# Netflix/metaflow

Measured on AMD Instinct MI355X. Metric: tokens/sec, higher is better.
Workload: dtype bf16; 1 GPU; model=llama3-8b, global_batch=8, seq_len=4096, parallelism=dp1

## Files before the change

### metaflow_amd/ops/csrc/attention.hip

```cpp

#include "common.h"

#define ATT_D 128

typedef __attribute__((ext_vector_type(16))) float f16f;

DEV f16f mfma32(bf16x8 a, bf16x8 b, f16f c) {
  return __builtin_amdgcn_mfma_f32_32x32x16_bf16(a, b, c, 0, 0, 0);
}

struct WaveCoord {
  int wid, lane, l32, hi;
};

DEV WaveCoord wave_coord() {
  WaveCoord c;
  c.wid = threadIdx.x / WAVE;
  c.lane = threadIdx.x & (WAVE - 1);
  c.l32 = c.lane & 31;
  c.hi = c.lane >> 5;
  return c;
}

DEV int c_row(int r, int hi) { return (r & 3) + 8 * (r >> 2) + 4 * hi; }

DEV unsigned int pack_bf2(float lo, float hi) {
  union { __hip_bfloat162 h; unsigned int u; } c;
  c.h = __float22bfloat162_rn(make_float2(lo, hi));
  return c.u;
}

template <int NT>
DEV void col_to_afrags(const f16f* st, bf16x8* pa, int hi) {
  unsigned int pk[NT * 8], xp[NT * 8];
#pragma unroll
  for (int t = 0; t < NT; ++t)
#pragma unroll
    for (int j2 = 0; j2 < 8; ++j2)
      pk[t * 8 + j2] = pack_bf2(st[t][j2 * 2], st[t][j2 * 2 + 1]);
#pragma unroll
  for (int i = 0; i < NT * 8; ++i) xp[i] = __shfl_xor(pk[i], 32, WAVE);
#pragma unroll
  for (int ks = 0; ks < NT * 2; ++ks) {
    union {
      unsigned int w[4];
      bf16x8 v;
    } u;
    if (hi == 0) {
      u.w[0] = pk[4 * ks];
      u.w[1] = pk[4 * ks + 1];
      u.w[2] = xp[4 * ks];
      u.w[3] = xp[4 * ks + 1];
    } else {
      u.w[0] = xp[4 * ks + 2];
      u.w[1] = xp[4 * ks + 3];
      u.w[2] = pk[4 * ks + 2];
      u.w[3] = pk[4 * ks + 3];
    }
    pa[ks] = u.v;
  }
}


template <int ROWS, int BLOCK>
DEV void stage_panel(short* dst, const short* src,
                     long long src_row_stride) {
  constexpr int TOT = ROWS * 16;
#pragma unroll
  for (int it = 0; it < (TOT + BLOCK - 1) / BLOCK; ++it) {
    const int idx = it * BLOCK + threadIdx.x;
    if (idx < TOT) {
      const int r = idx % ROWS, c8 = idx / ROWS;
      bf16x8 v = *(const bf16x8*)(src + r * src_row_stride + c8 * 8);
      *(bf16x8*)(dst + (c8 >> 1) * (ROWS * 16) + r * 16 + (c8 & 1) * 8) =
          v;
    }
  }
}

template <int ROWS>
DEV bf16x8 frag8_panel(const short* tile, int row, int d0) {
  return *(const bf16x8*)(tile + (d0 >> 4) * (ROWS * 16) + row * 16
                          + (d0 & 15));
}

DEV unsigned long long tr_read(const short* lds_ptr) {
  unsigned int addr = (unsigned int)(unsigned long long)lds_ptr;
  unsigned long long out;
  asm volatile("ds_read_b64_tr_b16 %0, %1" : "=v"(out) : "v"(addr));
  return out;
}

union BFrag {
  unsigned long long u[2];
  bf16x8 v;
};

template <int ROWS>
DEV void tr_load_bfrags(BFrag bfr[4], const short* tile, int row0,
                        int lane, int hi) {
  const int tr_lane_off = (((lane >> 2) & 3) * 16) + (lane & 3) * 4;
  const int tr_panel = ((lane >> 4) & 1) * (ROWS * 16);
#pragma unroll
  for (int n = 0; n < 4; ++n) {
    const int base = n * 2 * (ROWS * 16) + tr_panel
                     + (row0 + hi * 8) * 16 + tr_lane_off;
    bfr[n].u[0] = tr_read(tile + base);
    bfr[n].u[1] = tr_read(tile + base + 4 * 16);
  }
}

DEV void put_elem(short* p, float x) { *p = f2bf(x); }
DEV void put_elem(float* p, float x) { *p = x; }

template <bool ROW_SCALE, typename T>
DEV void store_acc_tile(T* dst, long long off0, int row0, const f16f acc[4],
                        int l32, int hi, float lane_scale = 1.f) {
#pragma unroll
  for (int r = 0; r < 16; ++r) {
    const int row_local = c_row(r, hi);
    float f = 1.f;
    if (ROW_SCALE) f = __shfl(lane_scale, row_local + 32 * hi, WAVE);
    const long long obase = off0 + (long long)(row0 + row_local) * ATT_D;
#pragma unroll
    for (int n = 0; n < 4; ++n)
      put_elem(dst + obase + n * 32 + l32,
               ROW_SCALE ? acc[n][r] * f : acc[n][r]);
  }
}


template <int BLOCK>
__global__ __launch_bounds__(512) void attn_fwd_v2_kernel(
    const short* __restrict__ q, const short* __restrict__ k,
    const short* __restrict__ v, short* __restrict__ o,
    float* __restrict__ lse, int B, int H, int Hkv, int S, float scale,
    int causal) {
  constexpr int BQ = 256, BKV = 64;
  __shared__ short kp[2][BKV * ATT_D];
  __shared__ short vp[2][BKV * ATT_D];

  const int qb = blockIdx.x;
  const int h = blockIdx.y;
  const int b = blockIdx.z;
  const int hk = h / (H / Hkv);
  const WaveCoord c = wave_coord();
  const int wid = c.wid, lane = c.lane, l32 = c.l32, hi = c.hi;

  const int my_qrow = qb * BQ + wid * 32 + l32;
  const long long hoff = ((long long)b * H + h) * S;
  const long long qoff = (hoff + qb * BQ) * ATT_D;
  const long long kvoff0 = ((long long)b * Hkv + hk) * S * ATT_D;

  bf16x8 q_reg[8];
  {
    const short* qrow = q + (hoff + my_qrow) * ATT_D;
#pragma unroll
    for (int s = 0; s < 8; ++s)
      q_reg[s] = *(const bf16x8*)(qrow + s * 16 + hi * 8);
  }

  float m_run = -INFINITY;
  float l_run = 0.f;
  f16f acc_o[4];
#pragma unroll
  for (int n = 0; n < 4; ++n) acc_o[n] = (f16f){};

  const int tid = threadIdx.x;
  bf16x8 stg_k[2], stg_v[2];
  int stg_r[2], stg_c8[2];
#pragma unroll
  for (int u = 0; u < 2; ++u) {
    const int idx = u * BLOCK + tid;
    stg_r[u] = idx / 16;
    stg_c8[u] = idx % 16;
  }

#define MFX_STAGE_LOAD(jj)                                               \
  {                                                                      \
    const short* kb_ = k + kvoff0 + (long long)(jj) * BKV * ATT_D;       \
    const short* vb_ = v + kvoff0 + (long long)(jj) * BKV * ATT_D;       \
    _Pragma("unroll") for (int u = 0; u < 2; ++u) {                      \
      stg_k[u] = *(const bf16x8*)(kb_ + stg_r[u] * ATT_D + stg_c8[u] * 8);\
      stg_v[u] = *(const bf16x8*)(vb_ + stg_r[u] * ATT_D + stg_c8[u] * 8);\
    }                                                                    \
  }

#define MFX_STAGE_WRITE(buf)                                             \
  {                                                                      \
    _Pragma("unroll") for (int u = 0; u < 2; ++u) {                      \
      const int pel_ = (stg_c8[u] >> 1) * (BKV * 16) + stg_r[u] * 16     \
                       + (stg_c8[u] & 1) * 8;                            \
      *(bf16x8*)(kp[buf] + pel_) = stg_k[u];                             \
      *(bf16x8*)(vp[buf] + pel_) = stg_v[u];                             \
    }                                                                    \
  }

  const int kv_tiles =
      causal ? (qb * BQ + BQ) / BKV : S / BKV;
  MFX_STAGE_LOAD(0);
  MFX_STAGE_WRITE(0);
  __syncthreads();
  for (int j = 0; j < kv_tiles; ++j) {
    const int cur = j & 1;
    if (j + 1 < kv_tiles) MFX_STAGE_LOAD(j + 1);

    const bool active = !causal || (j * BKV <= qb * BQ + wid * 32 + 31);
    if (active) {

    f16f st[2];
#pragma unroll
    for (int t = 0; t < 2; ++t) {
      st[t] = (f16f){};
#pragma unroll
      for (int s = 0; s < 8; ++s) {
        bf16x8 kf = frag8_panel<BKV>(kp[cur], t * 32 + l32,
                                     s * 16 + hi * 8);
        st[t] = mfma32(kf, q_reg[s], st[t]);
      }
    }

    const bool diag = causal && (j * BKV + BKV > qb * BQ);
    float pmax = -INFINITY;
#pragma unroll
    for (int t = 0; t < 2; ++t) {
#pragma unroll
      for (int r = 0; r < 16; ++r) {
        float sv = st[t][r] * scale;
        if (diag) {
          const int kvg = j * BKV + t * 32 + c_row(r, hi);
          if (kvg > my_qrow) sv = -INFINITY;
        }
        st[t][r] = sv;
        pmax = fmaxf(pmax, sv);
      }
    }
    pmax = fmaxf(pmax, __shfl_xor(pmax, 32, WAVE));
    const float newm = fmaxf(m_run, pmax);
    const float rescale = __expf(m_run - newm);
    m_run = newm;

    float psum = 0.f;
#pragma unroll
    for (int t = 0; t < 2; ++t)
#pragma unroll
      for (int r = 0; r < 16; ++r) {
        float e = __expf(st[t][r] - newm);
        st[t][r] = e;
        psum += e;
      }
    psum += __shfl_xor(psum, 32, WAVE);
    l_run = l_run * rescale + psum;

    {
#pragma unroll
      for (int r = 0; r < 16; ++r) {
        const float f = __shfl(rescale, c_row(r, hi) + 32 * hi, WAVE);
#pragma unroll
        for (int n = 0; n < 4; ++n) acc_o[n][r] *= f;
      }
    }

    bf16x8 pa[4];
    col_to_afrags<2>(st, pa, hi);

    {
      const int tr_lane_off = (((lane >> 2) & 3) * 16) + (lane & 3) * 4;
      const int tr_panel = ((lane >> 4) & 1) * (BKV * 16);
#pragma unroll
      for (int ks = 0; ks < 4; ++ks) {
        BFrag bfr[4];
#pragma unroll
        for (int n = 0; n < 4; ++n) {
          const int base = n * 2 * (BKV * 16) + tr_panel
                           + (ks * 16 + hi * 8) * 16 + tr_lane_off;
          bfr[n].u[0] = tr_read(vp[cur] + base);
          bfr[n].u[1] = tr_read(vp[cur] + base + 4 * 16);
        }
        asm volatile("s_waitcnt lgkmcnt(0)");
        __builtin_amdgcn_sched_barrier(0);
#pragma unroll
        for (int n = 0; n < 4; ++n)
          acc_o[n] = mfma32(pa[ks], bfr[n].v, acc_o[n]);
      }
    }
    }

    if (j + 1 < kv_tiles) MFX_STAGE_WRITE(cur ^ 1);
    __syncthreads();
  }
#undef MFX_STAGE_LOAD
#undef MFX_STAGE_WRITE

  float inv_l = 1.f / l_run;
  store_acc_tile<true>(o, qoff, wid * 32, acc_o, l32, hi, inv_l);
  if (hi == 0)
    lse[hoff + my_qrow] = m_run + __logf(l_run);
}

__global__ void attn_bwd_delta_kernel(const short* __restrict__ dout,
                                      const short* __restrict__ o,
                                      float* __restrict__ delta,
                                      long long rows) {
  const int lane = threadIdx.x & (WAVE - 1);
  const int wid = threadIdx.x / WAVE;
  const long long row = (long long)blockIdx.x * (blockDim.x / WAVE) + wid;
  if (row >= rows) return;
  const short* dr = dout + row * ATT_D;
  const short* orow = o + row * ATT_D;
  float s = bf2f(dr[lane]) * bf2f(orow[lane])
            + bf2f(dr[lane + 64]) * bf2f(orow[lane + 64]);
  s = wave_sum(s);
  if (lane == 0) delta[row] = s;
}


template <int BLOCK>
__global__ __launch_bounds__(512) void attn_bwd_dq_v2_kernel(
    const short* __restrict__ q, const short* __restrict__ k,
    const short* __restrict__ v, const short* __restrict__ dout,
    const float* __restrict__ lse, const float* __restrict__ delta,
    short* __restrict__ dq, int B, int H, int Hkv, int S, float scale,
    int causal) {
  constexpr int BQ = 256, BKV = 64;
  __shared__ short kp[BKV * ATT_D];
  __shared__ short vp[BKV * ATT_D];

  const int qb = blockIdx.x;
  const int h = blockIdx.y;
  const int b = blockIdx.z;
  const int hk = h / (H / Hkv);
  const int wid = threadIdx.x / WAVE;
  const int lane = threadIdx.x & (WAVE - 1);
  const int l32 = lane & 31;
  const int hi = lane >> 5;

  const int my_qrow = qb * BQ + wid * 32 + l32;
  const long long hoff = ((long long)b * H + h) * S;
  const long long qoff = (hoff + qb * BQ) * ATT_D;
  const long long kvoff0 = ((long long)b * Hkv + hk) * S * ATT_D;

  bf16x8 q_reg[8], do_reg[8];
  {
    const short* qrow = q + (hoff + my_qrow) * ATT_D;
    const short* drow = dout + (hoff + my_qrow) * ATT_D;
#pragma unroll
    for (int s = 0; s < 8; ++s) {
      q_reg[s] = *(const bf16x8*)(qrow + s * 16 + hi * 8);
      do_reg[s] = *(const bf16x8*)(drow + s * 16 + hi * 8);
    }
  }
  const float my_lse = lse[hoff + my_qrow];
  const float my_del = delta[hoff + my_qrow];

  f16f acc_dq[4];
#pragma unroll
  for (int n = 0; n < 4; ++n) acc_dq[n] = (f16f){};

  const int kv_tiles = causal ? (qb * BQ + BQ) / BKV : S / BKV;
  for (int j = 0; j < kv_tiles; ++j) {
    __syncthreads();
    stage_panel<BKV, BLOCK>(kp, k + kvoff0 + (long long)j * BKV * ATT_D,
                            ATT_D);
    stage_panel<BKV, BLOCK>(vp, v + kvoff0 + (long long)j * BKV * ATT_D,
                            ATT_D);
    __syncthreads();
    if (causal && j * BKV > qb * BQ + wid * 32 + 31) continue;

#pragma unroll
    for (int t = 0; t < 2; ++t) {
      f16f st = (f16f){}, dpt = (f16f){};
#pragma unroll
      for (int s = 0; s < 8; ++s) {
        bf16x8 kf = frag8_panel<BKV>(kp, t * 32 + l32, s * 16 + hi * 8);
        bf16x8 vf = frag8_panel<BKV>(vp, t * 32 + l32, s * 16 + hi * 8);
        st = mfma32(kf, q_reg[s], st);
        dpt = mfma32(vf, do_reg[s], dpt);
      }
#pragma unroll
      for (int r = 0; r < 16; ++r) {
        const int kvg = j * BKV + t * 32 + c_row(r, hi);
        float p = 0.f;
        if (!causal || kvg <= my_qrow)
          p = __expf(st[r] * scale - my_lse);
        st[r] = p * (dpt[r] - my_del) * scale;
      }
      bf16x8 pa[2];
      col_to_afrags<1>(&st, pa, hi);
#pragma unroll
      for (int ks = 0; ks < 2; ++ks) {
        BFrag bfr[4];
        tr_load_bfrags<BKV>(bfr, kp, t * 32 + ks * 16, lane, hi);
        asm volatile("s_waitcnt lgkmcnt(0)");
        __builtin_amdgcn_sched_barrier(0);
#pragma unroll
        for (int n = 0; n < 4; ++n)
          acc_dq[n] = mfma32(pa[ks], bfr[n].v, acc_dq[n]);
      }
    }
  }

#pragma unroll
  for (int r = 0; r < 16; ++r) {
    const int row_local = (r & 3) + 8 * (r >> 2) + 4 * hi;
    const long long obase =
        qoff + (long long)(wid * 32 + row_local) * ATT_D;
#pragma unroll
    for (int n = 0; n < 4; ++n)
      dq[obase + n * 32 + l32] = f2bf(acc_dq[n][r]);
  }
}


DEV void acc_to_bfrags(const f16f& x, bf16x8* pb) {
#pragma unroll
  for (int s = 0; s < 2; ++s) {
    unsigned int w[4];
#pragma unroll
    for (int i = 0; i < 4; ++i)
      w[i] = pack_bf2(x[8 * s + 2 * i], x[8 * s + 2 * i + 1]);
    union {
      unsigned int w[4];
      bf16x8 v;
    } u;
#pragma unroll
    for (int i = 0; i < 2; ++i) {
      auto r = __builtin_amdgcn_permlane32_swap(w[i], w[2 + i], false,
                                                false);
      u.w[i] = r[0];
      u.w[2 + i] = r[1];
    }
    pb[s] = u.v;
  }
}

DEV void lds_wave_fence() {
  __builtin_amdgcn_fence(__ATOMIC_RELEASE, "wavefront");
  __builtin_amdgcn_wave_barrier();
  __builtin_amdgcn_fence(__ATOMIC_ACQUIRE, "wavefront");
}

DEV void store_acc_tile_t(float* dst, long long off0, float* tw,
                          const f16f acc[4], int l32, int hi) {
#pragma unroll
  for (int n = 0; n < 4; ++n) {
#pragma unroll
    for (int r = 0; r < 16; ++r) {
      const int dl = (r & 3) + 8 * (r >> 2) + 4 * hi;
      tw[l32 * 32 + (dl ^ l32)] = acc[n][r];
    }
    lds_wave_fence();
#pragma unroll
    for (int i = 0; i < 16; ++i) {
      const int row = 2 * i + hi;
      dst[off0 + (long long)row * ATT_D + n * 32 + l32] =
          tw[row * 32 + (l32 ^ row)];
    }
    lds_wave_fence();
  }
}

extern __shared__ __attribute__((aligned(16))) short dkdv_v_img[];
#define DKDV_DYN_LDS (256 * ATT_D * 2)

template <int BLOCK>
__global__ __launch_bounds__(512) void attn_bwd_dkdv_v2_kernel(
    const short* __restrict__ q, const short* __restrict__ k,
    const short* __restrict__ v, const short* __restrict__ dout,
    const float* __restrict__ lse, const float* __restrict__ delta,
    float* __restrict__ dk_part, float* __restrict__ dv_part,
    int B, int H, int Hkv, int S, float scale, int causal) {
  constexpr int BKVB = 256, BQ2 = 64;
  __shared__ short qp[BQ2 * ATT_D];
  __shared__ short dop[BQ2 * ATT_D];
  __shared__ float lse_s[BQ2];
  __shared__ float del_s[BQ2];

  const int kvb = blockIdx.x;
  const int h = blockIdx.y;
  const int b = blockIdx.z;
  const int G = H / Hkv;
  const int hk = h / G;
  const int wid = threadIdx.x / WAVE;
  const int lane = threadIdx.x & (WAVE - 1);
  const int l32 = lane & 31;
  const int hi = lane >> 5;

  const int my_kvrow = kvb * BKVB + wid * 32 + l32;
  const long long kvoff =
      (((long long)b * Hkv + hk) * S + kvb * BKVB) * ATT_D;

  bf16x8 kr[8];
  short* vimg = dkdv_v_img + wid * (32 * ATT_D) + lane * 8;
  {
    const short* krow = k + kvoff + (long long)(wid * 32 + l32) * ATT_D;
    const short* vrow = v + kvoff + (long long)(wid * 32 + l32) * ATT_D;
#pragma unroll
    for (int s = 0; s < 8; ++s) {
      kr[s] = *(const bf16x8*)(krow + s * 16 + hi * 8);
      *(bf16x8*)(vimg + s * 512) = *(const bf16x8*)(vrow + s * 16 + hi * 8);
    }
#pragma unroll
    for (int s = 0; s < 8; ++s) asm volatile("" : "+v"(kr[s]));
  }

  f16f acc_dk[4], acc_dv[4];
#pragma unroll
  for (int n = 0; n < 4; ++n) {
    acc_dk[n] = (f16f){};
    acc_dv[n] = (f16f){};
  }

  const long long hoff = ((long long)b * H + h) * S;
  const int jq0 = causal ? (kvb * BKVB) / BQ2 : 0;
  const int nq = S / BQ2;
  for (int jq = jq0; jq < nq; ++jq) {
    __syncthreads();
    const short* qsrc = q + (hoff + (long long)jq * BQ2) * ATT_D;
    const short* dsrc = dout + (hoff + (long long)jq * BQ2) * ATT_D;
    stage_panel<BQ2, BLOCK>(qp, qsrc, ATT_D);
    stage_panel<BQ2, BLOCK>(dop, dsrc, ATT_D);
    if (threadIdx.x < BQ2) {
      lse_s[threadIdx.x] = lse[hoff + jq * BQ2 + threadIdx.x];
      del_s[threadIdx.x] = delta[hoff + jq * BQ2 + threadIdx.x];
    }
    __syncthreads();
    if (causal && jq * BQ2 + BQ2 - 1 < kvb * BKVB + wid * 32) continue;

#pragma unroll
    for (int t = 0; t < 2; ++t) {
      f16f st = (f16f){}, dpt = (f16f){};
#pragma unroll
      for (int s = 0; s < 8; ++s) {
        bf16x8 qf = frag8_panel<BQ2>(qp, t * 32 + l32, s * 16 + hi * 8);
        bf16x8 df = frag8_panel<BQ2>(dop, t * 32 + l32, s * 16 + hi * 8);
        bf16x8 vf = *(const bf16x8*)(vimg + s * 512);
        st = mfma32(qf, kr[s], st);
        dpt = mfma32(df, vf, dpt);
      }
#pragma unroll
      for (int g = 0; g < 4; ++g) {
        const int q0l = t * 32 + g * 8 + 4 * hi;
        const f32x4 lv = *(const f32x4*)&lse_s[q0l];
        const f32x4 dl = *(const f32x4*)&del_s[q0l];
#pragma unroll
        for (int j = 0; j < 4; ++j) {
          const int r = g * 4 + j;
          const int qrg = jq * BQ2 + q0l + j;
          float p = 0.f;
          if (!causal || qrg >= my_kvrow)
            p = __expf(st[r] * scale - lv[j]);
          st[r] = p;
          dpt[r] = p * (dpt[r] - dl[j]) * scale;
        }
      }
      bf16x8 pb[2], pbk[2];
      acc_to_bfrags(st, pb);
      BFrag bfr[2][4];
      const int tr_lane_off = (((lane >> 2) & 3) * 16) + (lane & 3) * 4;
      const int tr_panel = ((lane >> 4) & 1) * (BQ2 * 16);
      const short* g_tile[4] = {dop, dop, qp, qp};
      int g_q0[4];
      g_q0[0] = t * 32;
      g_q0[1] = t * 32 + 16;
      g_q0[2] = t * 32;
      g_q0[3] = t * 32 + 16;
#pragma unroll
      for (int n = 0; n < 4; ++n) {
        const int base = n * 2 * (BQ2 * 16) + tr_panel
                         + (g_q0[0] + hi * 8) * 16 + tr_lane_off;
        bfr[0][n].u[0] = tr_read(g_tile[0] + base);
        bfr[0][n].u[1] = tr_read(g_tile[0] + base + 4 * 16);
      }
      acc_to_bfrags(dpt, pbk);
#pragma unroll
      for (int g = 0; g < 4; ++g) {
        const int cur = g & 1;
        if (g < 3) {
#pragma unroll
          for (int n = 0; n < 4; ++n) {
            const int base = n * 2 * (BQ2 * 16) + tr_panel
                             + (g_q0[g + 1] + hi * 8) * 16 + tr_lane_off;
            bfr[cur ^ 1][n].u[0] = tr_read(g_tile[g + 1] + base);
            bfr[cur ^ 1][n].u[1] = tr_read(g_tile[g + 1] + base + 4 * 16);
          }
          asm volatile("s_waitcnt lgkmcnt(8)");
        } else {
          asm volatile("s_waitcnt lgkmcnt(0)");
        }
        __builtin_amdgcn_sched_barrier(0);
        const bf16x8 bop = (g < 2) ? pb[g] : pbk[g - 2];
        f16f* acc = (g < 2) ? acc_dv : acc_dk;
#pragma unroll
        for (int n = 0; n < 4; ++n)
          acc[n] = mfma32(bfr[cur][n].v, bop, acc[n]);
      }
    }
  }

  __syncthreads();
  float* tw = (float*)(wid < 4 ? qp : dop) + (wid & 3) * 1024;
  const long long poff =
      (hoff + (long long)kvb * BKVB + wid * 32) * ATT_D;
  store_acc_tile_t(dk_part, poff, tw, acc_dk, l32, hi);
  store_acc_tile_t(dv_part, poff, tw, acc_dv, l32, hi);
}

__global__ void dkdv_reduce_kernel(const float* __restrict__ dk_part,
                                   const float* __restrict__ dv_part,
                                   short* __restrict__ dk,
                                   short* __restrict__ dv,
                                   long long n4_kv, int G,
                                   long long head_elems) {
  const long long stride = (long long)gridDim.x * blockDim.x;
  for (long long i4 = (long long)blockIdx.x * blockDim.x + threadIdx.x;
       i4 < n4_kv; i4 += stride) {
    const long long i = i4 * 4;
    const long long slot = i / head_elems;
    const long long rem = i - slot * head_elems;
    const float* kp = dk_part + slot * G * head_elems + rem;
    const float* vp = dv_part + slot * G * head_elems + rem;
    f32x4 ks = *(const f32x4*)kp;
    f32x4 vs = *(const f32x4*)vp;
    for (int g = 1; g < G; ++g) {
      const f32x4 k2 = *(const f32x4*)(kp + (long long)g * head_elems);
      const f32x4 v2 = *(const f32x4*)(vp + (long long)g * head_elems);
#pragma unroll
      for (int j = 0; j < 4; ++j) {
        ks[j] += k2[j];
        vs[j] += v2[j];
      }
    }
    bf16x4 ko, vo;
// ... 10 lines not shown
```

### metaflow_amd/ops/csrc/mfx_hip.hip

```cpp

#include <torch/extension.h>
#include <hip/hip_runtime.h>
#include <c10/hip/HIPStream.h>

#include <vector>

#include "elementwise.hip"
#include "adam.hip"
#include "cross_entropy.hip"
#include "attention.hip"
#include "append.hip"
#include "decode.hip"
#include "paged.hip"
#include "append_paged.hip"
#include "debug_kernels.hip"

namespace {

constexpr int kBlock = 256;
constexpr int kGridCap = 2048;

inline hipStream_t cur_stream() {
  return c10::hip::getCurrentHIPStream().stream();
}
// ... 144 lines not shown
  auto du = torch::empty_like(u);
  long long n8 = g.numel() / 8;
  swiglu_bwd_kernel<<<grid_for(n8), kBlock, 0, cur_stream()>>>(
      bf(g), bf(u), bf(dy), bfm(dg), bfm(du), n8);
  HIP_CHECK_KERNEL();
  return {dg, du};
}

std::vector<torch::Tensor> swiglu_gu_fwd(torch::Tensor gu) {
  check_bf16(gu, "gu");
  const int I2 = gu.size(-1);
  TORCH_CHECK(I2 % 16 == 0, "fused swiglu needs 2I % 16 == 0");
  const int I = I2 / 2;
  const long long rows = gu.numel() / I2;
  auto sizes = gu.sizes().vec();
  sizes.back() = I;
  auto y = torch::empty(sizes, gu.options());
  long long total = rows * (I / 8);
  swiglu_gu_fwd_kernel<<<grid_for(total), kBlock, 0, cur_stream()>>>(
      bf(gu), bfm(y), rows, I);
  HIP_CHECK_KERNEL();
  return {y};
}

torch::Tensor swiglu_gu_bwd(torch::Tensor gu, torch::Tensor dy) {
  const int I = gu.size(-1) / 2;
  const long long rows = gu.numel() / (2 * I);
  auto dgu = torch::empty_like(gu);
  long long total = rows * (I / 8);
  swiglu_gu_bwd_kernel<<<grid_for(total), kBlock, 0, cur_stream()>>>(
      bf(gu), bf(dy.contiguous()), bfm(dgu), rows, I);
  HIP_CHECK_KERNEL();
  return dgu;
}

torch::Tensor decode_tokens_u16(torch::Tensor x) {
  TORCH_CHECK(x.is_cuda() && x.is_contiguous());
  TORCH_CHECK(x.scalar_type() == torch::kUInt8, "pass raw bytes (uint8)");
  TORCH_CHECK(x.numel() % 16 == 0,
              "token buffer must hold a multiple of 8 uint16 tokens");
  const long long n = x.numel() / 2;
  auto y = torch::empty({n}, x.options().dtype(torch::kInt64));
  decode_tokens_u16_kernel<<<grid_for(n / 8), kBlock, 0, cur_stream()>>>(
      reinterpret_cast<const unsigned short*>(x.data_ptr()),
      reinterpret_cast<long long*>(y.data_ptr<int64_t>()), n / 8);
  HIP_CHECK_KERNEL();
  return y;
}

torch::Tensor quant_e4m3(torch::Tensor x, double scale) {
  check_bf16(x, "x");
  TORCH_CHECK(x.numel() % 8 == 0, "quant_e4m3 needs numel % 8 == 0");
  auto y = torch::empty_like(x, x.options().dtype(torch::kUInt8));
  long long n8 = x.numel() / 8;
  quant_e4m3_kernel<<<grid_for(n8), kBlock, 0, cur_stream()>>>(
      bf(x), y.data_ptr<unsigned char>(), (float)scale, n8);
  HIP_CHECK_KERNEL();
  return y;
}

torch::Tensor quant_e5m2(torch::Tensor x, double scale) {
  check_bf16(x, "x");
  TORCH_CHECK(x.numel() % 8 == 0, "quant_e5m2 needs numel % 8 == 0");
  auto y = torch::empty_like(x, x.options().dtype(torch::kUInt8));
  long long n8 = x.numel() / 8;
  quant_e5m2_kernel<<<grid_for(n8), kBlock, 0, cur_stream()>>>(
      bf(x), y.data_ptr<unsigned char>(), (float)scale, n8);
  HIP_CHECK_KERNEL();
  return y;
}

torch::Tensor add_bf16(torch::Tensor a, torch::Tensor b) {
  check_bf16(a, "a");
  TORCH_CHECK(a.numel() % 8 == 0);
  auto y = torch::empty_like(a);
  long long n8 = a.numel() / 8;
  add_bf16_kernel<<<grid_for(n8), kBlock, 0, cur_stream()>>>(
      bf(a), bf(b), bfm(y), n8);
  HIP_CHECK_KERNEL();
  return y;
}

void adamw(torch::Tensor p, torch::Tensor g, torch::Tensor m, torch::Tensor v,
           c10::optional<torch::Tensor> master, double lr, double beta1,
           double beta2, double eps, double weight_decay, long step,
           double grad_scale) {
  const long long n = p.numel();
  float bias_c1 = 1.f / (1.f - powf((float)beta1, (float)step));
  float bias_c2 = 1.f / (1.f - powf((float)beta2, (float)step));
  if (p.scalar_type() == torch::kBFloat16) {
    TORCH_CHECK(n % 4 == 0, "bf16 adamw requires numel % 4 == 0");
    float* master_ptr =
        master.has_value() ? master->data_ptr<float>() : nullptr;
    adamw_kernel<<<grid_for(n / 4), kBlock, 0, cur_stream()>>>(
        bfm(p), bf(g), m.data_ptr<float>(), v.data_ptr<float>(), master_ptr,
        n, (float)lr, (float)beta1, (float)beta2, (float)eps,
        (float)weight_decay, bias_c1, bias_c2, (float)grad_scale);
    HIP_CHECK_KERNEL();
  } else {
    adamw_f32_kernel<<<grid_for(n), kBlock, 0, cur_stream()>>>(
        p.data_ptr<float>(), g.data_ptr<float>(), m.data_ptr<float>(),
        v.data_ptr<float>(), n, (float)lr, (float)beta1, (float)beta2,
        (float)eps, (float)weight_decay, bias_c1, bias_c2,
        (float)grad_scale);
    HIP_CHECK_KERNEL();
  }
}

std::vector<torch::Tensor> cross_entropy_fwd(torch::Tensor logits,
                                             torch::Tensor targets,
                                             long ignore_index) {
  check_bf16(logits, "logits");
  const int V = logits.size(-1);
  const long long N = logits.numel() / V;
  auto loss = torch::empty({N}, logits.options().dtype(torch::kFloat32));
  auto rmax = torch::empty({N}, logits.options().dtype(torch::kFloat32));
  auto rlse = torch::empty({N}, logits.options().dtype(torch::kFloat32));
  int grid = (int)std::min<long long>(N, kGridCap);
  cross_entropy_fwd_kernel<kBlock><<<grid, kBlock, 0, cur_stream()>>>(
      bf(logits), reinterpret_cast<const long long*>(targets.data_ptr<int64_t>()), loss.data_ptr<float>(),
      rmax.data_ptr<float>(), rlse.data_ptr<float>(), N, V,
      (long long)ignore_index);
  HIP_CHECK_KERNEL();
  return {loss, rlse};
}

torch::Tensor cross_entropy_bwd(torch::Tensor logits, torch::Tensor targets,
                                torch::Tensor row_lse, torch::Tensor dloss,
                                long ignore_index) {
  const int V = logits.size(-1);
  const long long N = logits.numel() / V;
  auto dlogits = torch::empty_like(logits);
  int grid = (int)std::min<long long>(N, kGridCap);
  cross_entropy_bwd_kernel<kBlock><<<grid, kBlock, 0, cur_stream()>>>(
      bf(logits), reinterpret_cast<const long long*>(targets.data_ptr<int64_t>()), row_lse.data_ptr<float>(),
      dloss.data_ptr<float>(), bfm(dlogits), N, V, (long long)ignore_index);
  HIP_CHECK_KERNEL();
  return dlogits;
}

std::vector<torch::Tensor> attn_fwd(torch::Tensor q, torch::Tensor k,
                                    torch::Tensor v, double scale,
                                    bool causal) {
  check_bf16(q, "q");
  check_bf16(k, "k");
  check_bf16(v, "v");
  const int B = q.size(0), H = q.size(1), S = q.size(2), D = q.size(3);
  const int Hkv = k.size(1);
  TORCH_CHECK(D == 128, "attention requires head dim 128");
  TORCH_CHECK(S % 256 == 0, "attention kernel requires seqlen % 256 == 0");
  TORCH_CHECK(H % Hkv == 0, "GQA requires H % Hkv == 0");
  auto o = torch::empty_like(q);
  auto lse = torch::empty({B, H, S}, q.options().dtype(torch::kFloat32));
  dim3 grid(S / 256, H, B);
  attn_fwd_v2_kernel<512><<<grid, 512, 0, cur_stream()>>>(
      bf(q), bf(k), bf(v), bfm(o), lse.data_ptr<float>(), B, H, Hkv, S,
      (float)scale, causal ? 1 : 0);
  HIP_CHECK_KERNEL();
  return {o, lse};
}

std::vector<torch::Tensor> attn_bwd(torch::Tensor q, torch::Tensor k,
                                    torch::Tensor v, torch::Tensor o,
                                    torch::Tensor dout, torch::Tensor lse,
                                    double scale, bool causal) {
  check_bf16(q, "q");
  check_bf16(k, "k");
  check_bf16(v, "v");
  check_bf16(o, "o");
  check_bf16(dout, "dout");
  const int B = q.size(0), H = q.size(1), S = q.size(2), D = q.size(3);
  const int Hkv = k.size(1);
  TORCH_CHECK(D == 128, "attention requires head dim 128");
  TORCH_CHECK(S % 256 == 0, "attention kernel requires seqlen % 256 == 0");
  TORCH_CHECK(H % Hkv == 0, "GQA requires H % Hkv == 0");
  TORCH_CHECK(lse.is_cuda() && lse.scalar_type() == torch::kFloat32 &&
                  lse.is_contiguous(),
              "lse must be contiguous fp32 on GPU");
  TORCH_CHECK(lse.dim() == 3 && lse.size(0) == B && lse.size(1) == H &&
                  lse.size(2) == S,
              "lse must have shape [B,H,S]");
  auto dq = torch::empty_like(q);
  auto dk = torch::empty_like(k);
  auto dv = torch::empty_like(v);
  auto f32opts = q.options().dtype(torch::kFloat32);
  auto delta = torch::empty({B, H, S}, f32opts);
  auto dk_part = torch::empty({B, H, S, 128}, f32opts);
  auto dv_part = torch::empty({B, H, S, 128}, f32opts);
  const int icausal = causal ? 1 : 0;
  const dim3 grid(S / 256, H, B);

  {
    const long long rows = (long long)B * H * S;
    const int rows_per_block = kBlock / 64;
    const long long blocks = (rows + rows_per_block - 1) / rows_per_block;
    attn_bwd_delta_kernel<<<(int)blocks, kBlock, 0, cur_stream()>>>(
        bf(dout), bf(o), delta.data_ptr<float>(), rows);
    HIP_CHECK_KERNEL();
  }
  {
    static bool lds_set[64] = {};
    int dev_id = 0;
    TORCH_CHECK(hipGetDevice(&dev_id) == hipSuccess && dev_id < 64,
                "attn_bwd: hipGetDevice failed");
    if (!lds_set[dev_id]) {
      hipError_t e = hipFuncSetAttribute(
          reinterpret_cast<const void*>(&attn_bwd_dkdv_v2_kernel<512>),
          hipFuncAttributeMaxDynamicSharedMemorySize, DKDV_DYN_LDS);
      TORCH_CHECK(e == hipSuccess, "attn_bwd: cannot raise dynamic LDS: ",
                  hipGetErrorString(e));
      lds_set[dev_id] = true;
    }
  }
  attn_bwd_dkdv_v2_kernel<512><<<grid, 512, DKDV_DYN_LDS, cur_stream()>>>(
      bf(q), bf(k), bf(v), bf(dout), lse.data_ptr<float>(),
      delta.data_ptr<float>(), dk_part.data_ptr<float>(),
      dv_part.data_ptr<float>(), B, H, Hkv, S, (float)scale, icausal);
  HIP_CHECK_KERNEL();
  {
    const long long n4_kv = (long long)B * Hkv * S * 128 / 4;
    const long long head_elems = (long long)S * 128;
    int blocks = (int)std::min<long long>(
        (n4_kv + kBlock - 1) / kBlock, kGridCap);
    dkdv_reduce_kernel<<<blocks, kBlock, 0, cur_stream()>>>(
        dk_part.data_ptr<float>(), dv_part.data_ptr<float>(), bfm(dk),
        bfm(dv), n4_kv, H / Hkv, head_elems);
    HIP_CHECK_KERNEL();
  }
  attn_bwd_dq_v2_kernel<512><<<grid, 512, 0, cur_stream()>>>(
      bf(q), bf(k), bf(v), bf(dout), lse.data_ptr<float>(),
      delta.data_ptr<float>(), bfm(dq), B, H, Hkv, S, (float)scale,
      icausal);
  HIP_CHECK_KERNEL();
  return {dq, dk, dv};
}

torch::Tensor attn_decode_varlen(torch::Tensor q, torch::Tensor kc,
                                 torch::Tensor vc, torch::Tensor lengths,
                                 long max_len, double scale) {
  check_bf16(q, "q");
  check_bf16(kc, "kc");
  check_bf16(vc, "vc");
  const int B = q.size(0), H = q.size(1);
  const int Hkv = kc.size(1), Lmax = kc.size(2);
  TORCH_CHECK(q.size(2) == 1 && q.size(3) == 128,
              "decode expects q [B,H,1,128]");
  TORCH_CHECK(kc.size(3) == 128 && max_len >= 1 && max_len <= Lmax);
  TORCH_CHECK(H % Hkv == 0);
  TORCH_CHECK(lengths.is_cuda() &&
              lengths.scalar_type() == torch::kInt32 &&
              lengths.numel() == B, "lengths must be int32 [B] on GPU");
  int splits = (int)std::max<long>(1, 1024 / ((long)B * H));
  splits = (int)std::min<long>(splits, (max_len + 255) / 256);
  splits = std::max(splits, 1);
  auto f32 = q.options().dtype(torch::kFloat32);
  auto o_part = torch::empty({splits, B, H, 128}, f32);
  auto ml_part = torch::empty({splits, B, H, 2}, f32);
  auto o = torch::empty_like(q);
  dim3 grid(splits, H, B);
  attn_decode_partial_kernel<<<grid, 256, 0, cur_stream()>>>(
      bf(q), bf(kc), bf(vc), lengths.data_ptr<int>(),
      o_part.data_ptr<float>(), ml_part.data_ptr<float>(), B, H, Hkv,
      Lmax, splits, (float)scale);
  HIP_CHECK_KERNEL();
  attn_decode_merge_kernel<<<B * H, 64, 0, cur_stream()>>>(
      o_part.data_ptr<float>(), ml_part.data_ptr<float>(), bfm(o), B, H,
      splits);
  HIP_CHECK_KERNEL();
  return o;
}

torch::Tensor attn_decode(torch::Tensor q, torch::Tensor kc,
                          torch::Tensor vc, long L, double scale) {
  auto lengths = torch::full({q.size(0)}, (long)L,
                             q.options().dtype(torch::kInt32));
  return attn_decode_varlen(q, kc, vc, lengths, L, scale);
}

torch::Tensor attn_append(torch::Tensor q, torch::Tensor kc,
                          torch::Tensor vc, torch::Tensor pos,
                          long max_len, double scale) {
  check_bf16(q, "q");
  check_bf16(kc, "kc");
  check_bf16(vc, "vc");
  TORCH_CHECK(q.dim() == 4 && q.size(3) == 128 && q.size(2) >= 1,
              "append expects q [B,H,Sq,128]");
  const int B = q.size(0), H = q.size(1), Sq = q.size(2);
  TORCH_CHECK(kc.dim() == 4 && kc.size(0) == B && kc.size(3) == 128,
              "append expects k_cache [B,Hkv,Lmax,128]");
  TORCH_CHECK(vc.sizes() == kc.sizes(),
              "k_cache and v_cache must have the same shape");
  const int Hkv = kc.size(1), Lmax = kc.size(2);
  TORCH_CHECK(H % Hkv == 0, "GQA requires H % Hkv == 0");
  TORCH_CHECK(max_len >= 1 && max_len <= Lmax,
              "max_len must be in [1, Lmax]");
  TORCH_CHECK(pos.is_cuda() && pos.scalar_type() == torch::kInt32 &&
              pos.numel() == B && pos.is_contiguous(),
              "pos must be int32 [B] on GPU");
  const bool small = Sq <= 32;
  const int bq = small ? 32 : 128;
  const int q_tiles = (Sq + bq - 1) / bq;
  const long wgs = (long)B * H * q_tiles;
  int splits = (int)std::max<long>(1, (small ? 1024 : 512) / wgs);
  splits = (int)std::min<long>(splits, (max_len + 255) / 256);
  splits = std::max(splits, 1);
  auto o = torch::empty_like(q);
  auto f32 = q.options().dtype(torch::kFloat32);
  torch::Tensor o_part, ml_part;
  float* o_part_p = nullptr;
  float* ml_part_p = nullptr;
  if (splits > 1) {
    o_part = torch::empty({splits, B, H, Sq, 128}, f32);
    ml_part = torch::empty({splits, B, H, Sq, 2}, f32);
    o_part_p = o_part.data_ptr<float>();
    ml_part_p = ml_part.data_ptr<float>();
  }
  dim3 grid(q_tiles * splits, H, B);
  if (small)
    attn_append_kernel<1><<<grid, 64, 0, cur_stream()>>>(
        bf(q), bf(kc), bf(vc), pos.data_ptr<int>(), bfm(o), o_part_p,
        ml_part_p, B, H, Hkv, Sq, Lmax, splits, (float)scale);
  else
    attn_append_kernel<4><<<grid, 256, 0, cur_stream()>>>(
        bf(q), bf(kc), bf(vc), pos.data_ptr<int>(), bfm(o), o_part_p,
        ml_part_p, B, H, Hkv, Sq, Lmax, splits, (float)scale);
  HIP_CHECK_KERNEL();
  if (splits > 1) {
    const long long R = (long long)B * H * Sq;
    attn_append_merge_kernel<<<(int)((R + 3) / 4), 256, 0, cur_stream()>>>(
        o_part_p, ml_part_p, bfm(o), R, splits);
    HIP_CHECK_KERNEL();
  }
  return o;
}

void check_page_pool(const torch::Tensor& kp, const torch::Tensor& vp) {
  check_bf16(kp, "k_pages");
  check_bf16(vp, "v_pages");
  TORCH_CHECK(kp.dim() == 4 && kp.size(2) == PG_ROWS && kp.size(3) == PG_D,
              "page pool must be [num_pages, Hkv, 64, 128]");
  TORCH_CHECK(vp.sizes() == kp.sizes(),
              "k_pages and v_pages must have the same shape");
}

void check_block_table(const torch::Tensor& table, int B) {
  TORCH_CHECK(table.is_cuda() && table.scalar_type() == torch::kInt32 &&
              table.dim() == 2 && table.size(0) == B &&
              table.is_contiguous(),
              "block_table must be contiguous int32 [B, pages_per_seq] "
              "on GPU");
}

torch::Tensor attn_decode_paged(torch::Tensor q, torch::Tensor kp,
                                torch::Tensor vp, torch::Tensor table,
                                torch::Tensor lengths, long max_len,
                                double scale) {
  check_bf16(q, "q");
  check_page_pool(kp, vp);
  TORCH_CHECK(q.dim() == 4 && q.size(2) == 1 && q.size(3) == PG_D,
              "paged decode expects q [B,H,1,128]");
  const int B = q.size(0), H = q.size(1);
  const int num_pages = kp.size(0), Hkv = kp.size(1);
  TORCH_CHECK(H % Hkv == 0, "GQA requires H % Hkv == 0");
  check_block_table(table, B);
  const int table_stride = table.size(1);
  TORCH_CHECK(max_len >= 1 && max_len <= (long)table_stride * PG_ROWS,
              "max_len must be in [1, 64 * pages_per_seq]");
  TORCH_CHECK(lengths.is_cuda() &&
              lengths.scalar_type() == torch::kInt32 &&
              lengths.numel() == B && lengths.is_contiguous(),
              "lengths must be int32 [B] on GPU");
  int splits = (int)std::max<long>(1, 1024 / ((long)B * H));
  splits = (int)std::min<long>(splits, (max_len + 255) / 256);
  splits = (int)std::min<long>(splits,
                               (max_len + PG_ROWS - 1) / PG_ROWS);
  splits = std::max(splits, 1);
  auto f32 = q.options().dtype(torch::kFloat32);
  auto o_part = torch::empty({splits, B, H, 128}, f32);
  auto ml_part = torch::empty({splits, B, H, 2}, f32);
  auto o = torch::empty_like(q);
  dim3 grid(splits, H, B);
  attn_decode_paged_partial_kernel<<<grid, 256, 0, cur_stream()>>>(
// ... 179 lines not shown
```

Baseline: 18550 tokens/s.

## Reorder attention grids heavy-first, double-buffer dQ KV staging, transpose MFMA outputs

Flattens the attention grids to 1D and maps blocks so causal query tiles with the most KV work launch first, which is meant to reduce tail imbalance. The dQ backward kernel gains register-prefetched, double-buffered K/V staging through a second dynamic-LDS buffer, so global loads overlap compute and one barrier per tile is dropped. The forward and dQ kernels swap MFMA operands so P lands in B-fragments via permlane32_swap. That removes per-row shuffles for the rescale and half-wave reductions. Outputs are written as bf16 through an LDS transpose for coalesced 16-byte stores. In exchange the dQ kernel uses more LDS and the block-index mapping becomes more complex.

```diff
diff --git a/metaflow_amd/ops/csrc/attention.hip b/metaflow_amd/ops/csrc/attention.hip
--- a/metaflow_amd/ops/csrc/attention.hip
+++ b/metaflow_amd/ops/csrc/attention.hip
@@ -129,6 +129,98 @@
   }
 }
 
+DEV void acc_to_bfrags(const f16f& x, bf16x8* pb) {
+#pragma unroll
+  for (int s = 0; s < 2; ++s) {
+    unsigned int w[4];
+#pragma unroll
+    for (int i = 0; i < 4; ++i)
+      w[i] = pack_bf2(x[8 * s + 2 * i], x[8 * s + 2 * i + 1]);
+    union {
+      unsigned int w[4];
+      bf16x8 v;
+    } u;
+#pragma unroll
+    for (int i = 0; i < 2; ++i) {
+      auto r = __builtin_amdgcn_permlane32_swap(w[i], w[2 + i], false,
+                                                false);
+      u.w[i] = r[0];
+      u.w[2 + i] = r[1];
+    }
+    pb[s] = u.v;
+  }
+}
+
+DEV float half_pair_max(float x) {
+  const unsigned int u = __float_as_uint(x);
+  auto r = __builtin_amdgcn_permlane32_swap(u, u, false, false);
+  return fmaxf(__uint_as_float(r[0]), __uint_as_float(r[1]));
+}
+
+DEV float half_pair_sum(float x) {
+  const unsigned int u = __float_as_uint(x);
+  auto r = __builtin_amdgcn_permlane32_swap(u, u, false, false);
+  return __uint_as_float(r[0]) + __uint_as_float(r[1]);
+}
+
+DEV void lds_wave_fence() {
+  __builtin_amdgcn_fence(__ATOMIC_RELEASE, "wavefront");
+  __builtin_amdgcn_wave_barrier();
+  __builtin_amdgcn_fence(__ATOMIC_ACQUIRE, "wavefront");
+}
+
+template <int NB, bool ROW_SCALE>
+DEV void store_acc_tile_t_bf16(short* dst, long long off0, short* tw,
+                               const f16f acc[4], int lane,
+                               float lane_scale = 1.f) {
+  constexpr int SLOTS = NB * 4;
+  constexpr int ROWLEN = NB * 32;
+  const int l32 = lane & 31, hi = lane >> 5;
+#pragma unroll
+  for (int p = 0; p < 4 / NB; ++p) {
+#pragma unroll
+    for (int nb = 0; nb < NB; ++nb) {
+      const int n = p * NB + nb;
+#pragma unroll
+      for (int g = 0; g < 4; ++g) {
+        bf16x4 w;
+#pragma unroll
+        for (int j = 0; j < 4; ++j)
+          w[j] = f2bf(ROW_SCALE ? acc[n][4 * g + j] * lane_scale
+                                : acc[n][4 * g + j]);
+        const int slot = (nb * 4 + g) ^ (l32 & (SLOTS - 1));
+        *(bf16x4*)(tw + l32 * ROWLEN + slot * 8 + hi * 4) = w;
+      }
+    }
+    lds_wave_fence();
+#pragma unroll
+    for (int i = 0; i < SLOTS / 2; ++i) {
+      const int row = i * (64 / SLOTS) + lane / SLOTS;
+      const int c = lane & (SLOTS - 1);
+      const bf16x8 v = *(const bf16x8*)(tw + row * ROWLEN
+                                        + ((c ^ (row & (SLOTS - 1))) * 8));
+      *(bf16x8*)(dst + off0 + (long long)row * ATT_D + p * ROWLEN + c * 8) =
+          v;
+    }
+    if (p + 1 < 4 / NB) lds_wave_fence();
+  }
+}
+
+struct BlockCoord {
+  int rank, h, b;
+};
+
+DEV BlockCoord block_coord(int T, int H) {
+  const int bid = blockIdx.x;
+  const int per_b = T * H;
+  BlockCoord c;
+  c.b = bid / per_b;
+  const int r = bid - c.b * per_b;
+  c.rank = r / H;
+  c.h = r - c.rank * H;
+  return c;
+}
+
 
 template <int BLOCK>
 __global__ __launch_bounds__(512) void attn_fwd_v2_kernel(
@@ -140,9 +232,10 @@
   __shared__ short kp[2][BKV * ATT_D];
   __shared__ short vp[2][BKV * ATT_D];
 
-  const int qb = blockIdx.x;
-  const int h = blockIdx.y;
-  const int b = blockIdx.z;
+  const BlockCoord bc = block_coord(S / BQ, H);
+  const int qb = S / BQ - 1 - bc.rank;
+  const int h = bc.h;
+  const int b = bc.b;
   const int hk = h / (H / Hkv);
   const WaveCoord c = wave_coord();
   const int wid = c.wid, lane = c.lane, l32 = c.l32, hi = c.hi;
@@ -235,7 +328,7 @@
         pmax = fmaxf(pmax, sv);
       }
     }
-    pmax = fmaxf(pmax, __shfl_xor(pmax, 32, WAVE));
+    pmax = half_pair_max(pmax);
     const float newm = fmaxf(m_run, pmax);
     const float rescale = __expf(m_run - newm);
     m_run = newm;
@@ -249,20 +342,17 @@
         st[t][r] = e;
         psum += e;
       }
-    psum += __shfl_xor(psum, 32, WAVE);
+    psum = half_pair_sum(psum);
     l_run = l_run * rescale + psum;
 
-    {
-#pragma unroll
-      for (int r = 0; r < 16; ++r) {
-        const float f = __shfl(rescale, c_row(r, hi) + 32 * hi, WAVE);
-#pragma unroll
-        for (int n = 0; n < 4; ++n) acc_o[n][r] *= f;
-      }
-    }
-
-    bf16x8 pa[4];
-    col_to_afrags<2>(st, pa, hi);
+#pragma unroll
+    for (int n = 0; n < 4; ++n)
+#pragma unroll
+      for (int r = 0; r < 16; ++r) acc_o[n][r] *= rescale;
+
+    bf16x8 pb[4];
+    acc_to_bfrags(st[0], pb);
+    acc_to_bfrags(st[1], pb + 2);
 
     {
       const int tr_lane_off = (((lane >> 2) & 3) * 16) + (lane & 3) * 4;
@@ -281,7 +371,7 @@
         __builtin_amdgcn_sched_barrier(0);
 #pragma unroll
         for (int n = 0; n < 4; ++n)
-          acc_o[n] = mfma32(pa[ks], bfr[n].v, acc_o[n]);
+          acc_o[n] = mfma32(bfr[n].v, pb[ks], acc_o[n]);
       }
     }
     }
@@ -293,7 +383,9 @@
 #undef MFX_STAGE_WRITE
 
   float inv_l = 1.f / l_run;
-  store_acc_tile<true>(o, qoff, wid * 32, acc_o, l32, hi, inv_l);
+  short* tw = (wid < 4 ? &kp[0][0] : &vp[0][0]) + (wid & 3) * (32 * ATT_D);
+  store_acc_tile_t_bf16<4, true>(o, qoff + (long long)wid * 32 * ATT_D, tw,
+                                 acc_o, lane, inv_l);
   if (hi == 0)
     lse[hoff + my_qrow] = m_run + __logf(l_run);
 }
@@ -315,6 +407,9 @@
 }
 
 
+extern __shared__ __attribute__((aligned(16))) short dq_kv2[];
+#define DQ_DYN_LDS (2 * 64 * ATT_D * 2)
+
 template <int BLOCK>
 __global__ __launch_bounds__(512) void attn_bwd_dq_v2_kernel(
     const short* __restrict__ q, const short* __restrict__ k,
@@ -326,9 +421,10 @@
   __shared__ short kp[BKV * ATT_D];
   __shared__ short vp[BKV * ATT_D];
 
-  const int qb = blockIdx.x;
-  const int h = blockIdx.y;
-  const int b = blockIdx.z;
+  const BlockCoord bc = block_coord(S / BQ, H);
+  const int qb = S / BQ - 1 - bc.rank;
+  const int h = bc.h;
+  const int b = bc.b;
   const int hk = h / (H / Hkv);
   const int wid = threadIdx.x / WAVE;
   const int lane = threadIdx.x & (WAVE - 1);
@@ -357,23 +453,46 @@
 #pragma unroll
   for (int n = 0; n < 4; ++n) acc_dq[n] = (f16f){};
 
+  const int tid = threadIdx.x;
+  bf16x8 stg_k[2], stg_v[2];
+#define MFX_DQ_LOAD(jj)                                                  \
+  {                                                                      \
+    const short* kb_ = k + kvoff0 + (long long)(jj) * BKV * ATT_D;       \
+    const short* vb_ = v + kvoff0 + (long long)(jj) * BKV * ATT_D;       \
+    _Pragma("unroll") for (int u = 0; u < 2; ++u) {                      \
+      const int idx_ = u * BLOCK + tid;                                  \
+      stg_k[u] = *(const bf16x8*)(kb_ + (idx_ / 16) * ATT_D + (idx_ % 16) * 8);\
+      stg_v[u] = *(const bf16x8*)(vb_ + (idx_ / 16) * ATT_D + (idx_ % 16) * 8);\
+    }                                                                    \
+  }
+#define MFX_DQ_WRITE(buf)                                                \
+  {                                                                      \
+    _Pragma("unroll") for (int u = 0; u < 2; ++u) {                      \
+      const int idx_ = u * BLOCK + tid;                                  \
+      const int pel_ = ((idx_ % 16) >> 1) * (BKV * 16) + (idx_ / 16) * 16\
+                       + ((idx_ % 16) & 1) * 8;                          \
+      *(bf16x8*)(((buf) ? dq_kv2 : kp) + pel_) = stg_k[u];               \
+      *(bf16x8*)(((buf) ? dq_kv2 + BKV * ATT_D : vp) + pel_) = stg_v[u]; \
+    }                                                                    \
+  }
   const int kv_tiles = causal ? (qb * BQ + BQ) / BKV : S / BKV;
+  MFX_DQ_LOAD(0);
+  MFX_DQ_WRITE(0);
+  __syncthreads();
   for (int j = 0; j < kv_tiles; ++j) {
-    __syncthreads();
-    stage_panel<BKV, BLOCK>(kp, k + kvoff0 + (long long)j * BKV * ATT_D,
-                            ATT_D);
-    stage_panel<BKV, BLOCK>(vp, v + kvoff0 + (long long)j * BKV * ATT_D,
-                            ATT_D);
-    __syncthreads();
-    if (causal && j * BKV > qb * BQ + wid * 32 + 31) continue;
+    const int cur = j & 1;
+    const short* kpc = cur ? dq_kv2 : kp;
+    const short* vpc = cur ? dq_kv2 + BKV * ATT_D : vp;
+    if (j + 1 < kv_tiles) MFX_DQ_LOAD(j + 1);
+    if (!(causal && j * BKV > qb * BQ + wid * 32 + 31)) {
 
 #pragma unroll
     for (int t = 0; t < 2; ++t) {
       f16f st = (f16f){}, dpt = (f16f){};
 #pragma unroll
       for (int s = 0; s < 8; ++s) {
-        bf16x8 kf = frag8_panel<BKV>(kp, t * 32 + l32, s * 16 + hi * 8);
-        bf16x8 vf = frag8_panel<BKV>(vp, t * 32 + l32, s * 16 + hi * 8);
+        bf16x8 kf = frag8_panel<BKV>(kpc, t * 32 + l32, s * 16 + hi * 8);
+        bf16x8 vf = frag8_panel<BKV>(vpc, t * 32 + l32, s * 16 + hi * 8);
         st = mfma32(kf, q_reg[s], st);
         dpt = mfma32(vf, do_reg[s], dpt);
       }
@@ -385,60 +504,31 @@
           p = __expf(st[r] * scale - my_lse);
         st[r] = p * (dpt[r] - my_del) * scale;
       }
-      bf16x8 pa[2];
-      col_to_afrags<1>(&st, pa, hi);
+      bf16x8 pb[2];
+      acc_to_bfrags(st, pb);
 #pragma unroll
       for (int ks = 0; ks < 2; ++ks) {
         BFrag bfr[4];
-        tr_load_bfrags<BKV>(bfr, kp, t * 32 + ks * 16, lane, hi);
+        tr_load_bfrags<BKV>(bfr, kpc, t * 32 + ks * 16, lane, hi);
         asm volatile("s_waitcnt lgkmcnt(0)");
         __builtin_amdgcn_sched_barrier(0);
 #pragma unroll
         for (int n = 0; n < 4; ++n)
-          acc_dq[n] = mfma32(pa[ks], bfr[n].v, acc_dq[n]);
-      }
-    }
-  }
-
-#pragma unroll
-  for (int r = 0; r < 16; ++r) {
-    const int row_local = (r & 3) + 8 * (r >> 2) + 4 * hi;
-    const long long obase =
-        qoff + (long long)(wid * 32 + row_local) * ATT_D;
-#pragma unroll
-    for (int n = 0; n < 4; ++n)
-      dq[obase + n * 32 + l32] = f2bf(acc_dq[n][r]);
-  }
-}
-
-
-DEV void acc_to_bfrags(const f16f& x, bf16x8* pb) {
-#pragma unroll
-  for (int s = 0; s < 2; ++s) {
-    unsigned int w[4];
-#pragma unroll
-    for (int i = 0; i < 4; ++i)
-      w[i] = pack_bf2(x[8 * s + 2 * i], x[8 * s + 2 * i + 1]);
-    union {
-      unsigned int w[4];
-      bf16x8 v;
-    } u;
-#pragma unroll
-    for (int i = 0; i < 2; ++i) {
-      auto r = __builtin_amdgcn_permlane32_swap(w[i], w[2 + i], false,
-                                                false);
-      u.w[i] = r[0];
-      u.w[2 + i] = r[1];
-    }
-    pb[s] = u.v;
-  }
-}
-
-DEV void lds_wave_fence() {
-  __builtin_amdgcn_fence(__ATOMIC_RELEASE, "wavefront");
-  __builtin_amdgcn_wave_barrier();
-  __builtin_amdgcn_fence(__ATOMIC_ACQUIRE, "wavefront");
-}
+          acc_dq[n] = mfma32(bfr[n].v, pb[ks], acc_dq[n]);
+      }
+    }
+    }
+    if (j + 1 < kv_tiles) MFX_DQ_WRITE(cur ^ 1);
+    __syncthreads();
+  }
+#undef MFX_DQ_LOAD
+#undef MFX_DQ_WRITE
+
+  short* tw = (wid < 4 ? kp : vp) + (wid & 3) * (32 * 64);
+  store_acc_tile_t_bf16<2, false>(dq, qoff + (long long)wid * 32 * ATT_D,
+                                  tw, acc_dq, lane);
+}
+
 
 DEV void store_acc_tile_t(float* dst, long long off0, float* tw,
                           const f16f acc[4], int l32, int hi) {
@@ -476,9 +566,10 @@
   __shared__ float lse_s[BQ2];
   __shared__ float del_s[BQ2];
 
-  const int kvb = blockIdx.x;
-  const int h = blockIdx.y;
-  const int b = blockIdx.z;
+  const BlockCoord bc = block_coord(S / BKVB, H);
+  const int kvb = bc.rank;
+  const int h = bc.h;
+  const int b = bc.b;
   const int G = H / Hkv;
   const int hk = h / G;
   const int wid = threadIdx.x / WAVE;
diff --git a/metaflow_amd/ops/csrc/mfx_hip.hip b/metaflow_amd/ops/csrc/mfx_hip.hip
--- a/metaflow_amd/ops/csrc/mfx_hip.hip
+++ b/metaflow_amd/ops/csrc/mfx_hip.hip
@@ -320,7 +320,7 @@
   TORCH_CHECK(H % Hkv == 0, "GQA requires H % Hkv == 0");
   auto o = torch::empty_like(q);
   auto lse = torch::empty({B, H, S}, q.options().dtype(torch::kFloat32));
-  dim3 grid(S / 256, H, B);
+  dim3 grid((S / 256) * H * B);
   attn_fwd_v2_kernel<512><<<grid, 512, 0, cur_stream()>>>(
       bf(q), bf(k), bf(v), bfm(o), lse.data_ptr<float>(), B, H, Hkv, S,
       (float)scale, causal ? 1 : 0);
@@ -356,7 +356,7 @@
   auto dk_part = torch::empty({B, H, S, 128}, f32opts);
   auto dv_part = torch::empty({B, H, S, 128}, f32opts);
   const int icausal = causal ? 1 : 0;
-  const dim3 grid(S / 256, H, B);
+  const dim3 grid((S / 256) * H * B);
 
   {
     const long long rows = (long long)B * H * S;
@@ -375,6 +375,10 @@
       hipError_t e = hipFuncSetAttribute(
           reinterpret_cast<const void*>(&attn_bwd_dkdv_v2_kernel<512>),
           hipFuncAttributeMaxDynamicSharedMemorySize, DKDV_DYN_LDS);
+      if (e == hipSuccess)
+        e = hipFuncSetAttribute(
+            reinterpret_cast<const void*>(&attn_bwd_dq_v2_kernel<512>),
+            hipFuncAttributeMaxDynamicSharedMemorySize, DQ_DYN_LDS);
       TORCH_CHECK(e == hipSuccess, "attn_bwd: cannot raise dynamic LDS: ",
                   hipGetErrorString(e));
       lds_set[dev_id] = true;
@@ -395,7 +399,7 @@
         bfm(dv), n4_kv, H / Hkv, head_elems);
     HIP_CHECK_KERNEL();
   }
-  attn_bwd_dq_v2_kernel<512><<<grid, 512, 0, cur_stream()>>>(
+  attn_bwd_dq_v2_kernel<512><<<grid, 512, DQ_DYN_LDS, cur_stream()>>>(
       bf(q), bf(k), bf(v), bf(dout), lse.data_ptr<float>(),
       delta.data_ptr<float>(), bfm(dq), B, H, Hkv, S, (float)scale,
       icausal);
```

Measured after the change: 21630 tokens/s (median of 6 runs). 16.6% higher.
